# CVLAB-Unibo/Real-time-self-adaptive-deep-stereo

Hardware: AMD Instinct MI355X
Metric: adapted stereo pairs/sec (whole node), MADNet full-backprop online adaptation 1242x375 (higher is better)
Workload: dtype bf16 MFMA operands, f32 accumulate/storage (forward: split-bf16 = 3 MFMAs per product on the large 3x3 layers, exact f32 MFMA on the others, so the disparity stays within 1e-3 px; gradients: plain bf16); 1 GPU; MADNet FULL adaptation step (fwd+SSIM/L1 loss+EPE+bwd+momentum), 1242x375, 1 pair/GPU/step, private model per stream; precision=mixed, launch=hipGraph replay, step_sync=stream, concurrent_private_streams_per_gpu=1

## Files before the change

real-time-self-adaptive-deep-stereo_amd/csrc/conv_patch.hip:

```cpp
#include "conv_args.h"
#include <stdlib.h>
#include <algorithm>
#include <atomic>

namespace {

struct PatchGeo {
    int TH, tiles_y, tiles_x, ntiles_n, nwg;
    int KP, CPT, PS;
    int nchunk;
    int patch_halfs;
    float inv_kp4;
    unsigned mul_kp8;
    int dbg;
    mh_tile_decode dec;
    mh_fastdiv f_kp4, f_pc;
    int xuse, per, n_major;
    mh_fastdiv f_pt;
};

constexpr int LSB = 80;
constexpr int PW = 18;

template <int WM, int WN, int MT, int NT, bool DGRAD, int CPTC = 0, bool X3 = false>
__global__ __launch_bounds__(WM * WN * 64) __attribute__((amdgpu_waves_per_eu(1, 2))) void conv_patch_kernel(ConvArgs p, PatchGeo g) {
    static_assert(!X3 || !DGRAD, "the split-bf16 instances are forward only");
    constexpr int NTH = WM * WN * 64;
    constexpr int BM = WM * MT * 16, BN = WN * NT * 16;
    constexpr int TH = BM / 16;
    HIP_DYNAMIC_SHARED(float, smem_all)
    unsigned short* const Ph = reinterpret_cast<unsigned short*>(smem_all);
    unsigned short* const Bh = Ph + (X3 ? 2 : 1) * g.patch_halfs;
    constexpr int BLO = 2 * BN * LSB;
    const int tid = threadIdx.x, lane = tid & 63, wave = tid >> 6;
    const int wm = wave / WN, wn = wave % WN;
    const int li = lane & 15, lq = lane >> 4;
    const int d = p.dil;

    const int lin = mh_xcd_remap(blockIdx.x, g.nwg);
    int tile_n, ttx, tty, cx, cy, b;
    mh_decode_tile(lin, g.dec, tile_n, ttx, tty, cx, cy, b);
    const int n0 = tile_n * BN;
    const int y00 = cy + d * (tty * TH), x00 = cx + d * (ttx * 16);

    const __amdgpu_buffer_rsrc_t rs_in = mh_make_rsrc(p.in, p.in_bytes);
    const __amdgpu_buffer_rsrc_t rs_w = mh_make_rsrc(p.w, p.w_bytes);

    constexpr int FU = 512 / NTH;
    constexpr int DI = (16 * BN) / NTH;
    constexpr int NB = DGRAD ? DI : 4 * FU;
    constexpr int NV = DGRAD ? DI : FU;
    float4 rb0[NB], rb1[NB];
    int voff[NV], vk[NV], vch[NV];
#pragma unroll
    for (int jj = 0; jj < NV; ++jj) {
        const int q = tid + NTH * jj;
        if (!DGRAD) {
            const int wi = q & 255;
            const int n4 = wi % (BN / 4), kq = wi / (BN / 4);
            const int n = n0 + n4 * 4;
            vch[jj] = __builtin_amdgcn_readfirstlane(q >> 8);
            vk[jj] = kq * 4;
            voff[jj] = (kq < 8 && n < p.N) ? (kq * 4 * p.N + n) * 4 : MH_OOB;
        } else {
            const int ch = q / (8 * BN), rem = q - ch * (8 * BN);
            const int nn = rem >> 3, kg = rem & 7;
            vch[jj] = ch;
            vk[jj] = kg * 4;
            voff[jj] = (n0 + nn < p.N) ? ((n0 + nn) * p.K + kg * 4) * 4 : MH_OOB;
        }
    }
// ... 561 lines not shown
            __builtin_amdgcn_sched_barrier(0);
        }
    }
    __syncthreads();

    constexpr int CS = BN + 4;
    float* const Cs = smem_all;
#pragma unroll
    for (int i = 0; i < MT; ++i)
#pragma unroll
        for (int j = 0; j < NT; ++j)
#pragma unroll
            for (int r = 0; r < 4; ++r)
                Cs[((wm * MT + i) * 16 + lq * 4 + r) * CS + wn * NT * 16 + j * 16 + li] = acc[i][j][r];
    __syncthreads();
    constexpr int C4 = BN / 4;
    constexpr int RP = NTH / C4;
    constexpr int PASSES = (BM + RP - 1) / RP;
    const __amdgpu_buffer_rsrc_t rs_out = mh_make_rsrc(p.out, p.out_bytes);
    const __amdgpu_buffer_rsrc_t rs_mask = mh_make_rsrc(p.mask_ref ? p.mask_ref : p.out, p.mask_ref ? p.mask_bytes : 0u);
    const int c4 = tid % C4;
    const int n = n0 + c4 * 4;
    float4 bv = make_float4(0.f, 0.f, 0.f, 0.f);
    if (p.bias && n < p.N) bv = *reinterpret_cast<const float4*>(p.bias + n);
#pragma unroll 4
    for (int ps = 0; ps < PASSES; ++ps) {
        const int row = tid / C4 + ps * RP;
        const int rr = row < BM ? row : 0;
        const int y = y00 + (rr >> 4) * d, x = x00 + (rr & 15) * d;
        const bool ok = (tid < RP * C4) && (row < BM) && (y < p.Ho) && (x < p.Wo) && (n < p.N);
        const int m = (b * p.Ho + y) * p.Wo + x;
        float4 v = *reinterpret_cast<const float4*>(&Cs[rr * CS + c4 * 4]);
        const int ooff = ok ? (m * p.out_ld + n) * 4 : MH_OOB;
        float4 old = make_float4(0.f, 0.f, 0.f, 0.f), mk = make_float4(1.f, 1.f, 1.f, 1.f);
        if (p.accumulate) old = mh_buf_load4(rs_out, ooff);
        if (p.mask_ref) mk = mh_buf_load4(rs_mask, ok ? (m * p.mask_ld + n) * 4 : MH_OOB);
        v.x += bv.x; v.y += bv.y; v.z += bv.z; v.w += bv.w;
        if (p.alpha != 1.0f) {
            v.x = v.x > 0.f ? v.x : p.alpha * v.x; v.y = v.y > 0.f ? v.y : p.alpha * v.y;
            v.z = v.z > 0.f ? v.z : p.alpha * v.z; v.w = v.w > 0.f ? v.w : p.alpha * v.w;
        }
        v.x += old.x; v.y += old.y; v.z += old.z; v.w += old.w;
        if (p.mask_ref) {
            v.x *= (mk.x > 0.f || n + 0 < p.mask_c0 || n + 0 >= p.mask_c1) ? 1.0f : p.mask_alpha;
            v.y *= (mk.y > 0.f || n + 1 < p.mask_c0 || n + 1 >= p.mask_c1) ? 1.0f : p.mask_alpha;
            v.z *= (mk.z > 0.f || n + 2 < p.mask_c0 || n + 2 >= p.mask_c1) ? 1.0f : p.mask_alpha;
            v.w *= (mk.w > 0.f || n + 3 < p.mask_c0 || n + 3 >= p.mask_c1) ? 1.0f : p.mask_alpha;
        }
        if (ok) *reinterpret_cast<float4*>(p.out + (int64_t)m * p.out_ld + n) = v;
        if (ok && p.shadow) *reinterpret_cast<uint2*>(p.shadow + (int64_t)m * p.shadow_ld + n) = make_uint2(mh_pack_bf16(v.x, v.y), mh_pack_bf16(v.z, v.w));
    }
}

template <bool DGRAD, int PL>
__global__ __launch_bounds__(1024) void conv_bank_small_kernel(ConvArgs p, PatchGeo g) {
    constexpr int NTH = 1024, TH = 2, BM = 32, BN = 32, MT = 2, NT = 2, NCH = 4;
    HIP_DYNAMIC_SHARED(float, smem_all)
    unsigned short* const Ph = reinterpret_cast<unsigned short*>(smem_all);
    const int tid = threadIdx.x, lane = tid & 63, wave = tid >> 6;
    const int li = lane & 15, lq = lane >> 4;
    const int d = p.dil;
    const int st = DGRAD ? 1 : p.stride;
    const int PC = st * 16 + 3 - st;

    int lin;
    if (g.xuse < 8) {
        const int xcd = (int)blockIdx.x & 7, idx = (int)blockIdx.x >> 3;
        lin = xcd * g.per + idx;
        if (xcd >= g.xuse || lin >= g.nwg) return;
    } else lin = mh_xcd_remap(blockIdx.x, g.nwg);
    int tile_n, ttx, tty, cx, cy, b;
    if (g.n_major) {
        const int tn = mh_fdiv(lin, g.f_pt);
        mh_decode_tile(lin - tn * (int)g.f_pt.d, g.dec, tile_n, ttx, tty, cx, cy, b);
        tile_n = tn;
    } else mh_decode_tile(lin, g.dec, tile_n, ttx, tty, cx, cy, b);
    const int n0 = tile_n * BN;
    const int y00 = cy + d * (tty * TH), x00 = cx + d * (ttx * 16);

    const __amdgpu_buffer_rsrc_t rs_in = mh_make_rsrc(p.in, p.in_bytes);
    const __amdgpu_buffer_rsrc_t rs_b = mh_make_rsrc(p.wb, p.wb_bytes);

    const int my_n = n0 + (tid & 31);
    const int my_row = tid >> 5;
    const int my_y = y00 + (my_row >> 4) * d, my_x = x00 + (my_row & 15) * d;
    const bool my_ok = my_y < p.Ho && my_x < p.Wo && my_n < p.N;
    const int64_t my_m = ((int64_t)b * p.Ho + my_y) * p.Wo + my_x;
    const __amdgpu_buffer_rsrc_t rs_bias = mh_make_rsrc(p.bias ? (const void*)p.bias : (const void*)p.in, p.bias ? (unsigned)(p.N * 4) : 0u);
    const __amdgpu_buffer_rsrc_t rs_old = mh_make_rsrc(p.out, p.accumulate ? p.out_bytes : 0u);
    const __amdgpu_buffer_rsrc_t rs_mk = mh_make_rsrc(p.mask_ref ? (const void*)p.mask_ref : (const void*)p.in, p.mask_ref ? p.mask_bytes : 0u);
    float my_bias, my_old, my_mk;
    const int np16 = (p.N + 15) >> 4;
    const int stride_b = np16 * PL * 1024;
    u32x4 fb[NCH][NT][PL];
#pragma unroll
    for (int c = 0; c < NCH; ++c) {
        const int q = wave + 16 * c;
#pragma unroll
        for (int j = 0; j < NT; ++j) {
            const int nt = tile_n * (BN / 16) + j;
            const int off = (q < g.nchunk && nt < np16) ? q * stride_b + nt * PL * 1024 + lane * 16 : MH_OOB;
#pragma unroll
            for (int pl = 0; pl < PL; ++pl) fb[c][j][pl] = __builtin_amdgcn_raw_buffer_load_b128(rs_b, off == MH_OOB ? MH_OOB : off + pl * 1024, 0, 0);
        }
    }

    {
        constexpr int U = 4, ROUNDS = 2;
        const int kp4 = g.KP >> 2;
        const int items = (st * TH + 3 - st) * PC * kp4;
        auto fdiv = [](int n, const mh_fastdiv& f) { const int h = (int)__umulhi((unsigned)n, f.m); return f.d > 1 ? h : n; };
#pragma unroll
        for (int rd = 0; rd < ROUNDS; ++rd) {
            if (rd > 0 && items <= rd * U * NTH) break;
            float4 wv[U];
            int ldsv[U], c4v[U];
#pragma unroll
            for (int u = 0; u < U; ++u) {
                const int q = tid + (rd * U + u) * NTH;
                const int pp = fdiv(q, g.f_kp4), c4 = q - pp * kp4;
                const int pi = fdiv(pp, g.f_pc), pj = pp - pi * PC;
                const int iy = y00 * st - p.pad_t + pi * d, ix = x00 * st - p.pad_l + pj * d;
                const bool ok = q < items && (unsigned)iy < (unsigned)p.Hi && (unsigned)ix < (unsigned)p.Wi && (c4 < p.G);
                int off = (((b * p.Hi + iy) * p.Wi + ix) * p.in_ld + c4 * 4) * 4;
                MH_KEEP_VGPR(off);
                wv[u] = mh_buf_load4(rs_in, ok ? off : MH_OOB);
                ldsv[u] = q < items ? pp * g.PS + c4 * 4 : -1;
                c4v[u] = c4;
            }
            if (rd == 0) {
                my_bias = mh_buf_load1(rs_bias, my_n < p.N ? my_n * 4 : MH_OOB);
                my_old = mh_buf_load1(rs_old, my_ok ? (int)((my_m * p.out_ld + my_n) * 4) : MH_OOB);
                my_mk = mh_buf_load1(rs_mk, my_ok ? (int)((my_m * p.mask_ld + my_n) * 4) : MH_OOB);
            }
#pragma unroll
            for (int u = 0; u < U; ++u) {
                float4 w = wv[u];
                const int c4 = c4v[u];
                w.y = (c4 * 4 + 1 < p.K) ? w.y : 0.f;
                w.z = (c4 * 4 + 2 < p.K) ? w.z : 0.f;
                w.w = (c4 * 4 + 3 < p.K) ? w.w : 0.f;
                const int lds = ldsv[u];
                if (lds >= 0) {
                    if constexpr (PL == 2) {
                        uint2 hi, lo;
                        mh_split_bf16x2(w.x, w.y, hi.x, lo.x);
                        mh_split_bf16x2(w.z, w.w, hi.y, lo.y);
                        *reinterpret_cast<uint2*>(Ph + lds) = hi;
                        *reinterpret_cast<uint2*>(Ph + g.patch_halfs + lds) = lo;
                    } else
                    *reinterpret_cast<uint2*>(Ph + lds) = make_uint2(mh_pack_bf16(w.x, w.y), mh_pack_bf16(w.z, w.w));
                }
            }
        }
    }
    __syncthreads();

    f32x4 acc[MT][NT];
#pragma unroll
    for (int i = 0; i < MT; ++i)
#pragma unroll
        for (int j = 0; j < NT; ++j) acc[i][j] = (f32x4){0.f, 0.f, 0.f, 0.f};
    const unsigned short* const Pw = Ph + (li * st) * g.PS + lq * 8;
#pragma unroll
    for (int c = 0; c < NCH; ++c) {
        const int q = wave + 16 * c;
        if (q < g.nchunk) {
            const int tap = q / g.CPT, c32 = q - tap * g.CPT;
            const int ky = tap / 3, kx = tap - ky * 3;
            const int oy = DGRAD ? 2 - ky : ky, ox = DGRAD ? 2 - kx : kx;
            const unsigned short* Ab = Pw + (oy * PC + ox) * g.PS + c32 * 32;
            u32x4 fa[MT][PL];
#pragma unroll
            for (int i = 0; i < MT; ++i)
#pragma unroll
                for (int pl = 0; pl < PL; ++pl) fa[i][pl] = *reinterpret_cast<const u32x4*>(Ab + pl * g.patch_halfs + (i * st) * PC * g.PS);
#pragma unroll
            for (int t = (PL == 2 ? 0 : 2); t < 3; ++t)
#pragma unroll
                for (int i = 0; i < MT; ++i)
#pragma unroll
                    for (int j = 0; j < NT; ++j)
                        acc[i][j] = mh_mfma_bf16(fa[i][t == 0 ? PL - 1 : 0], fb[c][j][t == 1 ? PL - 1 : 0], acc[i][j]);
        }
    }
    __syncthreads();
    constexpr int CS = BN + 1;
    float* const Cs = smem_all;
#pragma unroll
    for (int i = 0; i < MT; ++i)
#pragma unroll
        for (int j = 0; j < NT; ++j)
#pragma unroll
            for (int r = 0; r < 4; ++r)
                Cs[(wave * BM + i * 16 + lq * 4 + r) * CS + j * 16 + li] = acc[i][j][r];
    __syncthreads();
    {
        const int row = tid >> 5, col = tid & 31;
        float v = 0.f;
#pragma unroll
        for (int w = 0; w < 16; ++w) v += Cs[(w * BM + row) * CS + col];
        const int n = n0 + col;
        if (my_ok) {
            const int64_t m = my_m;
            v += my_bias;
            if (p.alpha != 1.0f) v = v > 0.f ? v : p.alpha * v;
            float* dst = p.out + m * p.out_ld + n;
            v += my_old;
            if (p.mask_ref) v *= (my_mk > 0.f || n < p.mask_c0 || n >= p.mask_c1) ? 1.0f : p.mask_alpha;
            *dst = v;
            if (p.shadow) p.shadow[m * p.shadow_ld + n] = (unsigned short)mh_pack_bf16(v, 0.f);
        }
    }
}

__global__ __launch_bounds__(256) void pack_weights_kernel(const mh_pack_seg* __restrict__ segs, int nseg) {
    const int lo = mh_find_seg(segs, nseg, (int)blockIdx.x);
    const mh_pack_seg sg = segs[lo];
    const int e = ((int)blockIdx.x - sg.blk0) * 256 + (int)threadIdx.x;
    const int lane = e & 63, qt = e >> 6;
    if (sg.trans == 2 || sg.trans == 3) {
        const int k16 = (sg.K + 15) >> 4, nt32 = (sg.N + 31) >> 5;
        const int kc = sg.kc16 > 0 ? sg.kc16 : k16, nch = (k16 + kc - 1) / kc;
        if (qt >= nch * sg.taps * kc * nt32) return;
        const int nt = qt % nt32, q = qt / nt32;
        const int st = q % kc, q2 = q / kc;
        const int tap = q2 % sg.taps, ch = q2 / sg.taps;
        const int k0 = (ch * kc + st) * 16 + (lane >> 5) * 8, n = nt * 32 + (lane & 31);
        const int ts = sg.trans == 3 ? sg.taps - 1 - tap : tap;
        float v[8];
#pragma unroll
        for (int j = 0; j < 8; ++j)
            v[j] = (k0 + j < sg.K && n < sg.N) ? (sg.trans == 3 ? sg.src[((int64_t)ts * sg.N + n) * sg.K + k0 + j] : sg.src[((int64_t)ts * sg.K + k0 + j) * sg.N + n]) : 0.f;
        unsigned hh[4], ll[4];
#pragma unroll
        for (int j = 0; j < 4; ++j) mh_split_bf16x2(v[2 * j], v[2 * j + 1], hh[j], ll[j]);
        const int pln = (sg.trans == 3 || sg.planes < 2) ? 1 : 2;
        u32x4* dst = reinterpret_cast<u32x4*>(sg.dst) + (int64_t)qt * (64 * pln) + lane;
        dst[0] = (u32x4){hh[0], hh[1], hh[2], hh[3]};
        if (pln == 2) dst[64] = (u32x4){ll[0], ll[1], ll[2], ll[3]};
        return;
    }
    const int cpt = (sg.K + 31) >> 5, np16 = (sg.N + 15) >> 4;
    if (qt >= sg.taps * cpt * np16) return;
    const int nt = qt % np16, q = qt / np16;
    const int c = q % cpt, tap = q / cpt;
    const int k0 = c * 32 + (lane >> 4) * 8, n = nt * 16 + (lane & 15);
    float v[8];
#pragma unroll
    for (int j = 0; j < 8; ++j)
        v[j] = (k0 + j < sg.K && n < sg.N) ? (sg.trans ? sg.src[((int64_t)tap * sg.N + n) * sg.K + k0 + j] : sg.src[((int64_t)tap * sg.K + k0 + j) * sg.N + n]) : 0.f;
    unsigned hh[4], ll[4];
#pragma unroll
    for (int j = 0; j < 4; ++j) mh_split_bf16x2(v[2 * j], v[2 * j + 1], hh[j], ll[j]);
    const u32x4 h = {hh[0], hh[1], hh[2], hh[3]}, l = {ll[0], ll[1], ll[2], ll[3]};
    u32x4* dst = reinterpret_cast<u32x4*>(sg.dst) + ((int64_t)qt * sg.planes) * 64 + lane;
    dst[0] = h;
    if (sg.planes > 1) dst[64] = l;
}

constexpr size_t PATCH_LDS_MAX = 150 * 1024;

size_t patch_lds(int TH, int BM, int BN, int KP, bool x3 = false) {
    const size_t tiles = ((size_t)(TH + 2) * PW * (KP + 16) * 2 + (size_t)2 * BN * LSB * 2) * (x3 ? 2 : 1);
    const size_t cs = (size_t)BM * (BN + 4) * 4;
    return tiles > cs ? tiles : cs;
}

size_t bank_lds(int TH, int BM, int BN, int KP, bool x3) {
    const size_t patch = (size_t)(TH + 2) * PW * (KP + 16) * 2 * (x3 ? 2 : 1);
    const size_t cs = (size_t)BM * (BN + 4) * 4;
    return patch > cs ? patch : cs;
}

constexpr int PATCH_DEFAULT = 1;
std::atomic<int> g_patch_mode{-2};
int patch_mode() {
    int m = g_patch_mode.load(std::memory_order_relaxed);
    if (m == -2) { const char* e = getenv("MH_CONV_PATCH"); m = e ? atoi(e) : PATCH_DEFAULT; g_patch_mode.store(m, std::memory_order_relaxed); }
    return m;
}
std::atomic<int> g_patch_launches{0};

template <int WM, int WN, int MT, int NT, bool DGRAD, int CPTC = 0, bool X3 = false>
int launch_patch(ConvArgs& a, hipStream_t s) {
    constexpr int BM = WM * MT * 16, BN = WN * NT * 16, TH = BM / 16;
    static std::atomic<uint64_t> attr_done{0};
    if (int rc = mh_lds_optin(attr_done, reinterpret_cast<const void*>(&conv_patch_kernel<WM, WN, MT, NT, DGRAD, CPTC, X3>), (int)PATCH_LDS_MAX, "conv_patch")) return rc;
    if (a.M < 0) return 0;
    PatchGeo g;
    g.TH = TH;
    const int d = a.dil;
    g.tiles_y = mh_cdiv(mh_cdiv(a.Ho, d), TH);
    g.tiles_x = mh_cdiv(mh_cdiv(a.Wo, d), 16);
    g.ntiles_n = mh_cdiv(a.N, BN);
    g.nwg = a.B * d * d * g.tiles_y * g.tiles_x * g.ntiles_n;
    {
        const int64_t nwg64 = (int64_t)g.nwg;
        const int dmax = std::max(std::max(g.ntiles_n, g.tiles_x), std::max(g.tiles_y, (int)d));
        MH_REQUIRE(mh_fastdiv_ok(nwg64, dmax), MH_ERR_UNSUPPORTED, "tile decode: %lld workgroups x divisor %d exceeds the 2^32 range of the magic-multiplier division", (long long)nwg64, dmax);
    }
    g.dec = mh_make_tile_decode(g.ntiles_n, g.tiles_x, g.tiles_y, d);
    g.KP = (a.K + 31) & ~31;
    g.CPT = g.KP / 32;
    g.PS = g.KP + 16;
    g.nchunk = 9 * g.CPT;
    g.patch_halfs = (TH + 2) * PW * g.PS;
    g.inv_kp4 = 1.0f / (float)(g.KP / 4);
    g.mul_kp8 = (unsigned)(((1ull << 32) + (g.KP / 8) - 1) / (g.KP / 8));
    g.dbg = (patch_mode() >> 9) & 3;
    const size_t lds = patch_lds(TH, BM, BN, g.KP, X3);
    ++g_patch_launches;
    mh_note_kernel("conv_patch_kernel<%d,%d,%d,%d,%s,CPTC=%d,%s> tile %dx%d K=%d dil=%d grid %d lds %d", WM, WN, MT, NT, DGRAD ? "dgrad" : "fwd", CPTC,
                   X3 ? "bf16x3" : "bf16", BM, BN, a.K, a.dil, g.nwg, (int)lds);
    hipLaunchKernelGGL((conv_patch_kernel<WM, WN, MT, NT, DGRAD, CPTC, X3>), dim3(g.nwg), dim3(WM * WN * 64), lds, s, a, g);
    return mh_check_launch("conv_patch");
}

std::atomic<int> g_bank_launches{0};
template <int WM, int WN, int MT, int NT, bool X3>
int launch_bank(ConvArgs& a, hipStream_t s) {
    constexpr int BM = WM * MT * 16, BN = WN * NT * 16, TH = BM / 16;
    static std::atomic<uint64_t> attr_done{0};
    if (int rc = mh_lds_optin(attr_done, reinterpret_cast<const void*>(&conv_bank_kernel<WM, WN, MT, NT, X3>), (int)PATCH_LDS_MAX, "conv_bank")) return rc;
    if (a.M < 0) return 0;
    PatchGeo g;
    g.TH = TH;
    const int d = a.dil;
    g.tiles_y = mh_cdiv(mh_cdiv(a.Ho, d), TH);
    g.tiles_x = mh_cdiv(mh_cdiv(a.Wo, d), 16);
    g.ntiles_n = mh_cdiv(a.N, BN);
    g.nwg = a.B * d * d * g.tiles_y * g.tiles_x * g.ntiles_n;
    {
        const int64_t nwg64 = (int64_t)g.nwg;
        const int dmax = std::max(std::max(g.ntiles_n, g.tiles_x), std::max(g.tiles_y, (int)d));
        MH_REQUIRE(mh_fastdiv_ok(nwg64, dmax), MH_ERR_UNSUPPORTED, "tile decode: %lld workgroups x divisor %d exceeds the 2^32 range of the magic-multiplier division", (long long)nwg64, dmax);
    }
    g.dec = mh_make_tile_decode(g.ntiles_n, g.tiles_x, g.tiles_y, d);
    g.KP = (a.K + 31) & ~31;
    g.CPT = g.KP / 32;
    g.PS = g.KP + 16;
    g.nchunk = 9 * g.CPT;
    g.patch_halfs = (TH + 2) * PW * g.PS;
    g.inv_kp4 = 1.0f / (float)(g.KP / 4);
    g.mul_kp8 = (unsigned)(((1ull << 32) + (g.KP / 8) - 1) / (g.KP / 8));
    g.dbg = (patch_mode() >> 9) & 3;
    const size_t lds = bank_lds(TH, BM, BN, g.KP, X3);
    ++g_patch_launches;
    ++g_bank_launches;
    mh_note_kernel("conv_bank_kernel<%d,%d,%d,%d,%s> tile %dx%d K=%d dil=%d grid %d lds %d", WM, WN, MT, NT, X3 ? "bf16x3" : "bf16", BM, BN, a.K, a.dil,
                   g.nwg, (int)lds);
    hipLaunchKernelGGL((conv_bank_kernel<WM, WN, MT, NT, X3>), dim3(g.nwg), dim3(WM * WN * 64), lds, s, a, g);
    return mh_check_launch("conv_bank");
}

std::atomic<int> g_bank_small_place{-1};
template <bool DGRAD, int PL>
int launch_bank_small(ConvArgs& a, hipStream_t s) {
    static std::atomic<uint64_t> attr_done{0};
    if (int rc = mh_lds_optin(attr_done, reinterpret_cast<const void*>(&conv_bank_small_kernel<DGRAD, PL>), (int)PATCH_LDS_MAX, "conv_bank_small")) return rc;
    if (a.M < 0) return 0;
    PatchGeo g;
    g.TH = 2;
    const int d = a.dil;
    g.tiles_y = mh_cdiv(mh_cdiv(a.Ho, d), 2);
    g.tiles_x = mh_cdiv(mh_cdiv(a.Wo, d), 16);
    g.ntiles_n = mh_cdiv(a.N, 32);
    g.nwg = a.B * d * d * g.tiles_y * g.tiles_x * g.ntiles_n;
    {
        const int64_t nwg64 = (int64_t)g.nwg;
        const int dmax = std::max(std::max(g.ntiles_n, g.tiles_x), std::max(g.tiles_y, (int)d));
        MH_REQUIRE(mh_fastdiv_ok(nwg64, dmax), MH_ERR_UNSUPPORTED, "tile decode: %lld workgroups x divisor %d exceeds the 2^32 range of the magic-multiplier division", (long long)nwg64, dmax);
    }
    g.KP = (a.K + 31) & ~31;
    {
        const int mode_raw = g_bank_small_place.load(std::memory_order_relaxed);
        const int mode = mode_raw < 0 ? 1 : mode_raw;
        const int npt = g.nwg / g.ntiles_n;
        int X = 8;
        if (mode >= 2) { X = 1; while (X < 8 && mh_cdiv(g.nwg, X) > 32) X *= 2; }
        const double bank = 9.0 * g.KP * a.N * 2.0 * PL, in = (double)a.B * (DGRAD ? a.Ho : a.Hi) * (DGRAD ? a.Wo : a.Wi) * a.K * 4.0;
        const double pix_major = X * bank + in;
        const double col_major = (double)std::max(X, g.ntiles_n) / g.ntiles_n * bank + std::min(X, g.ntiles_n) * in;
        g.n_major = (mode != 0 && mode != 2 && col_major < pix_major) ? 1 : 0;
        g.xuse = X;
        g.per = mh_cdiv(g.nwg, X);
        g.f_pt = mh_make_fastdiv(npt);
        MH_REQUIRE(mh_fastdiv_ok((int64_t)g.nwg, npt), MH_ERR_UNSUPPORTED, "tile decode: %d workgroups x %d pixel tiles exceeds the magic-multiplier range", g.nwg, npt);
    }
    g.dec = mh_make_tile_decode(g.n_major ? 1 : g.ntiles_n, g.tiles_x, g.tiles_y, d);
    g.CPT = g.KP / 32;
    g.PS = g.KP + 16;
    g.nchunk = 9 * g.CPT;
    const int st = DGRAD ? 1 : a.stride;
    g.patch_halfs = (st * 2 + 3 - st) * (st * 16 + 3 - st) * g.PS;
    g.f_kp4 = mh_make_fastdiv(g.KP / 4); g.f_pc = mh_make_fastdiv(st * 16 + 3 - st);
    g.inv_kp4 = 1.0f / (float)(g.KP / 4);
    g.mul_kp8 = (unsigned)(((1ull << 32) + (g.KP / 8) - 1) / (g.KP / 8));
    g.dbg = 0;
    const size_t patch = (size_t)g.patch_halfs * 2 * PL, cs = (size_t)16 * 32 * 33 * 4;
    const size_t lds = patch > cs ? patch : cs;
    ++g_bank_launches;
    const int nblocks = g.xuse < 8 ? 8 * g.per : g.nwg;
    mh_note_kernel("conv_bank_small_kernel<%s,%s> tile 32x32 K=%d N=%d dil=%d grid %d lds %d", DGRAD ? "dgrad" : "fwd", PL == 2 ? "bf16x3" : "bf16", a.K, a.N, a.dil,
                   g.nwg, (int)lds);
    hipLaunchKernelGGL((conv_bank_small_kernel<DGRAD, PL>), dim3(nblocks), dim3(1024), lds, s, a, g);
    return mh_check_launch("conv_bank_small");
}

template <int WM, int WN, int MT, int NT, bool DGRAD>
int launch_patch_k(ConvArgs& a, hipStream_t s) {
    const bool all = a.M < 0;
    const bool generic = !all && ((patch_mode() >> 11) & 1) != 0;
    int rc = 0;
    if constexpr (WM == 4) {
        if (all || (a.K == 128 && !generic)) { rc = launch_patch<WM, WN, MT, NT, DGRAD, 4>(a, s); if (!all || rc) return rc; }
        if (all || (a.K == 64 && !generic)) { rc = launch_patch<WM, WN, MT, NT, DGRAD, 2>(a, s); if (!all || rc) return rc; }
    }
    return launch_patch<WM, WN, MT, NT, DGRAD>(a, s);
}

template <int WM, int WN, int MT, bool DGRAD>
int launch_patch_n(ConvArgs& a, hipStream_t s, int bn) {
    const bool all = a.M < 0;
    int rc = 0;
    if (all || bn == 128) { rc = launch_patch_k<WM, WN, MT, 4, DGRAD>(a, s); if (!all || rc) return rc; }
    if (all || bn == 96) { rc = launch_patch_k<WM, WN, MT, 3, DGRAD>(a, s); if (!all || rc) return rc; }
    if (all || bn == 64) { rc = launch_patch_k<WM, WN, MT, 2, DGRAD>(a, s); if (!all || rc) return rc; }
    return rc;
}

int patch_bn(const ConvArgs& a) {
    if (a.N <= 32) return 32;
    return a.x3 ? (a.N > 64 ? 128 : 64) : (a.N > 96 ? 128 : (a.N > 64 ? 96 : 64));
}

int patch_bm(const ConvArgs& a) {
    if (a.x3) return a.N > 64 ? 64 : 128;
    if ((patch_mode() & 0xff) == 64 || (patch_mode() & 0xff) == 128) return patch_mode() & 0xff;
    return 128;
}
bool patch_w8(const ConvArgs& a) { return (patch_mode() & 0xff) == 1 ? true : (patch_mode() & 0x100) != 0; }

}

extern "C" int mh_tune_conv_patch(int mode) {
    g_patch_mode = mode < 0 ? PATCH_DEFAULT : mode;
    return g_patch_launches.exchange(0);
}

extern "C" int64_t mh_pack_bytes(int32_t taps, int32_t K, int32_t N, int32_t planes) {
    return (int64_t)taps * ((K + 31) / 32) * ((N + 15) / 16) * planes * 1024;
}
extern "C" int mh_pack_weights(const mh_pack_seg* segs_device, int32_t nseg, int32_t nblocks, void* stream) {
    MH_REQUIRE(segs_device && nseg > 0 && nblocks > 0, MH_ERR_ARG, "mh_pack_weights: empty segment table");
    hipLaunchKernelGGL(pack_weights_kernel, dim3(nblocks), dim3(256), 0, (hipStream_t)stream, segs_device, nseg);
    return mh_check_launch("pack_weights");
}
std::atomic<int> g_bank_small_maxpix{-2};
// ... 113 lines not shown
```

real-time-self-adaptive-deep-stereo_amd/madnet_hip/ops.py:

```python
import ctypes as C
import torch
from . import _ffi


def same_pad(in_size, k, stride=1, dilation=1):
    keff = (k - 1) * dilation + 1
    out = -(-in_size // stride)
    total = max((out - 1) * stride + keff - in_size, 0)
    return out, total // 2, total - total // 2


class View(object):
    __slots__ = ("t", "ptr", "B", "H", "W", "C", "ld")

    def __init__(self, t, B, H, W, C_, ld, coff=0):
        self.t, self.B, self.H, self.W, self.C, self.ld = t, B, H, W, C_, ld
        self.ptr = t.data_ptr() + 4 * coff

    @property
    def npix(self):
        return self.B * self.H * self.W

    def slice(self, c0, c1):
        v = View(self.t, self.B, self.H, self.W, c1 - c0, self.ld)
# ... 75 lines not shown
    return conv_desc(dx.B, Ho, Wo, dx.H, dx.W, cout, cin, kh, kw_, stride, dil, pt, pl, 1, 1, dz.ld, dx.ld,
                     precision=(_bwd_precision() if precision is None else precision), **kw)


def conv2d_takes_bank(qlib, x, w, out, stride, dil, mode, precision, mask_ref=None):
    d = (_dgrad_desc if mode else _fwd_desc)(x, w, out, stride, dil, precision, mask_ld=(mask_ref.ld if mask_ref is not None else 0))
    return qlib.conv2d_takes_bank(C.byref(d), _p(x), _p(w), _p(out), _p(mask_ref)) == 1


def conv2d_fwd(lib, x, w, b, out, stride=1, dil=1, alpha=1.0, accumulate=False, mask_ref=None, mask_alpha=1.0,
               mask_range=(0, 0), stream=None, precision=None, wb=None, shadow=None, out_planes=None):
    d = _fwd_desc(x, w, out, stride, dil, precision, alpha=alpha, mask_ld=(mask_ref.ld if mask_ref is not None else 0), accumulate=int(accumulate),
                  mask_alpha=mask_alpha, mask_c0=mask_range[0], mask_c1=mask_range[1])
    if out_planes is not None:
        assert (out_planes.B, out_planes.H, out_planes.W, out_planes.C) == (out.B, out.H, out.W, out.C)
        lib.conv2d_sh4(C.byref(d), _p(x), _p(w), _p(wb), _p(b), _p(out), _p(mask_ref), C.c_void_p(out_planes.hi.ptr), C.c_void_p(out_planes.lo.ptr), _p(stream))
    elif shadow is not None:
        assert (shadow.B, shadow.H, shadow.W, shadow.C) == (out.B, out.H, out.W, out.C)
        lib.conv2d_sh(C.byref(d), _p(x), _p(w), _p(wb), _p(b), _p(out), _p(mask_ref), C.c_void_p(shadow.ptr), _p(stream))
    elif wb is not None:
        lib.conv2d_wb(C.byref(d), _p(x), _p(w), _p(wb), _p(b), _p(out), _p(mask_ref), _p(stream))
    else:
        lib.conv2d(C.byref(d), _p(x), _p(w), _p(b), _p(out), _p(mask_ref), _p(stream))


PLANES_WHOLE_MAX = int(__import__("os").environ.get("MH_PLANES_WHOLE_MAX", "8"))


def planes_kc16(K):
    k16 = (K + 15) // 16
    return 0 if (k16 <= PLANES_WHOLE_MAX or k16 == 13) else 4


def check_planes_rule(qlib):
    for K in (16, 97, 112, 128, 129, 193, 208, 256, 385, 1025):
        if int(qlib.planes_kc16(K)) != planes_kc16(K):
            raise RuntimeError("libmadnet_hip: mh_planes_kc16(%d) = %d, host rule %d (MH_PLANES_WHOLE_MAX mismatch)" % (K, qlib.planes_kc16(K), planes_kc16(K)))


def _k16_padded(K):
    k16, kc = (K + 15) // 16, planes_kc16(K)
    return (k16 + kc - 1) // kc * kc if kc else k16


def pack_bytes(w, planes=2, trans=0):
    kh, kw, K, N = w.shape
    if trans == 2:
        return kh * kw * _k16_padded(K) * ((N + 31) // 32) * 1024 * planes
    if trans == 3:
        return kh * kw * _k16_padded(N) * ((K + 31) // 32) * 1024
    if trans:
        K, N = N, K
    return kh * kw * ((K + 31) // 32) * ((N + 15) // 16) * planes * 1024


def pack_weights(lib, pairs, device, keep, stream=None):
    if not pairs:
        return
    arr = (_ffi.PackSeg * len(pairs))()
    blk = 0
    for i, pr in enumerate(pairs):
        src, dst = pr[0], pr[1]
        planes = pr[2] if len(pr) > 2 else 2
        trans = pr[3] if len(pr) > 3 else 0
        kh, kw, K, N = src.shape
        if trans in (1, 3):
            K, N = N, K
        assert dst.numel() * dst.element_size() >= pack_bytes(src, planes, trans) and dst.data_ptr() % 16 == 0
        assert (trans != 3 or planes == 1)
        arr[i].src, arr[i].dst, arr[i].taps, arr[i].K, arr[i].N = src.data_ptr(), dst.data_ptr(), kh * kw, K, N
        arr[i].planes, arr[i].blk0, arr[i].trans = planes, blk, trans
        arr[i].kc16 = planes_kc16(K) if trans in (2, 3) else 0
        if trans in (2, 3):
            blk += (kh * kw * _k16_padded(K) * ((N + 31) // 32) * 64 + 255) // 256
        else:
            blk += (kh * kw * ((K + 31) // 32) * ((N + 15) // 16) * 64 + 255) // 256
    table = torch.frombuffer(bytearray(bytes(arr)), dtype=torch.uint8).to(device)
    keep.append(table)
    lib.pack_weights(C.c_void_p(table.data_ptr()), len(pairs), blk, _p(stream))


def conv2d_dgrad(lib, dz, w, dx, stride=1, dil=1, accumulate=False, mask_ref=None, mask_alpha=1.0, mask_range=(0, 0),
                 stream=None, wb=None, shadow=None, dz_shadow=None, mask_shadow=None):
    d = _dgrad_desc(dz, w, dx, stride, dil, None, mask_ld=(mask_ref.ld if mask_ref is not None else 0), accumulate=int(accumulate),
                    mask_alpha=mask_alpha, mask_c0=mask_range[0], mask_c1=mask_range[1])
    if dz_shadow is not None or mask_shadow is not None:
        assert dz_shadow is None or (dz_shadow.B, dz_shadow.H, dz_shadow.W, dz_shadow.C) == (dz.B, dz.H, dz.W, dz.C)
        assert mask_shadow is None or (mask_ref is not None and (mask_shadow.B, mask_shadow.H, mask_shadow.W, mask_shadow.C) == (dx.B, dx.H, dx.W, dx.C))
        assert shadow is None or (shadow.B, shadow.H, shadow.W, shadow.C) == (dx.B, dx.H, dx.W, dx.C)
        sp = lambda sh: C.c_void_p(sh.ptr) if sh is not None else None
        lib.conv2d_sh3(C.byref(d), _p(dz), sp(dz_shadow), _p(w), _p(wb), None, _p(dx), _p(mask_ref), sp(mask_shadow), sp(shadow), 0, _p(stream))
    elif shadow is not None:
        assert (shadow.B, shadow.H, shadow.W, shadow.C) == (dx.B, dx.H, dx.W, dx.C)
        lib.conv2d_sh(C.byref(d), _p(dz), _p(w), _p(wb), None, _p(dx), _p(mask_ref), C.c_void_p(shadow.ptr), _p(stream))
    elif wb is not None:
        lib.conv2d_wb(C.byref(d), _p(dz), _p(w), _p(wb), None, _p(dx), _p(mask_ref), _p(stream))
    else:
        lib.conv2d(C.byref(d), _p(dz), _p(w), None, _p(dx), _p(mask_ref), _p(stream))


def conv2d_wgrad(lib, x, dz, dw, db, stride=1, dil=1, stream=None):
    kh, kw, cin, cout = dw.shape
    Ho, Wo, pt, pl = conv_geometry(x.H, x.W, kh, kw, stride, dil)
    assert (dz.H, dz.W, dz.C) == (Ho, Wo, cout) and x.C == cin
    d = conv_desc(x.B, x.H, x.W, Ho, Wo, cin, cout, kh, kw, stride, dil, pt, pl, 0, 0, x.ld, dz.ld, precision=_bwd_precision())
    lib.conv2d_wgrad(C.byref(d), _p(x), _p(dz), dz.ld, _p(dw), _p(db), _p(stream))


class WgradWorkspace(object):
    CHUNK = 64 << 20

    def __init__(self, device):
        self.device = device
        self.chunks = []
        self.reset()

    def reset(self):
        self.ci, self.off = 0, 0

    def alloc(self, nfloats):
        nfloats = (nfloats + 3) // 4 * 4
        while True:
            if self.ci == len(self.chunks):
                self.chunks.append(torch.empty(max(self.CHUNK, nfloats), dtype=torch.float32, device=self.device))
                self.off = 0
            c = self.chunks[self.ci]
            if self.off + nfloats <= c.numel():
                p = c.data_ptr() + 4 * self.off
                self.off += nfloats
# ... 610 lines not shown
```

Measured before the change: 769.5 pairs/s.

## Tile weight packing through LDS and add an optional multi-tile bank_small kernel

The weight-pack kernel now stages 32x128 tiles of the f32 weights in shared memory, reading them with coalesced float4 loads when alignment allows, before splitting into bf16 hi/lo planes. Previously each thread gathered eight strided scalars, and in the transposed layouts those reads were poorly coalesced. Separately, the small-bank conv kernel is refactored into a per-tile device function. A MULTI variant can then keep the B fragments in registers and loop over several spatial tiles, capping the grid at one residency round. That variant is enabled only when a placement flag bit is set. The host block-count formula changes to match the new pack grid, and the two sides must stay in sync.

```diff
diff --git a/real-time-self-adaptive-deep-stereo_amd/csrc/conv_patch.hip b/real-time-self-adaptive-deep-stereo_amd/csrc/conv_patch.hip
--- a/real-time-self-adaptive-deep-stereo_amd/csrc/conv_patch.hip
+++ b/real-time-self-adaptive-deep-stereo_amd/csrc/conv_patch.hip
@@ -17,6 +17,8 @@
     mh_fastdiv f_kp4, f_pc;
     int xuse, per, n_major;
     mh_fastdiv f_pt;
+    int tiles;
+    mh_fastdiv f_grp;
 };
 
 constexpr int LSB = 80;
@@ -684,37 +686,21 @@
     }
 }
 
-template <bool DGRAD, int PL>
-__global__ __launch_bounds__(1024) void conv_bank_small_kernel(ConvArgs p, PatchGeo g) {
+template <bool DGRAD, int PL, bool REMAT = false>
+__device__ __forceinline__ void bank_small_tile(const ConvArgs& p, const PatchGeo& g, float* const smem_all, const u32x4 (&fb)[4][2][PL], const int n0, const int y00,
+                                                const int x00, const int b, const __amdgpu_buffer_rsrc_t rs_in) {
     constexpr int NTH = 1024, TH = 2, BM = 32, BN = 32, MT = 2, NT = 2, NCH = 4;
-    HIP_DYNAMIC_SHARED(float, smem_all)
     unsigned short* const Ph = reinterpret_cast<unsigned short*>(smem_all);
-    const int tid = threadIdx.x, lane = tid & 63, wave = tid >> 6;
-    const int li = lane & 15, lq = lane >> 4;
+    const int tid = threadIdx.x, wave = tid >> 6;
+    int stid = tid;
+    if constexpr (REMAT) MH_KEEP_VGPR(stid);
+    const int li = stid & 15, lq = (stid & 63) >> 4;
     const int d = p.dil;
     const int st = DGRAD ? 1 : p.stride;
     const int PC = st * 16 + 3 - st;
 
-    int lin;
-    if (g.xuse < 8) {
-        const int xcd = (int)blockIdx.x & 7, idx = (int)blockIdx.x >> 3;
-        lin = xcd * g.per + idx;
-        if (xcd >= g.xuse || lin >= g.nwg) return;
-    } else lin = mh_xcd_remap(blockIdx.x, g.nwg);
-    int tile_n, ttx, tty, cx, cy, b;
-    if (g.n_major) {
-        const int tn = mh_fdiv(lin, g.f_pt);
-        mh_decode_tile(lin - tn * (int)g.f_pt.d, g.dec, tile_n, ttx, tty, cx, cy, b);
-        tile_n = tn;
-    } else mh_decode_tile(lin, g.dec, tile_n, ttx, tty, cx, cy, b);
-    const int n0 = tile_n * BN;
-    const int y00 = cy + d * (tty * TH), x00 = cx + d * (ttx * 16);
-
-    const __amdgpu_buffer_rsrc_t rs_in = mh_make_rsrc(p.in, p.in_bytes);
-    const __amdgpu_buffer_rsrc_t rs_b = mh_make_rsrc(p.wb, p.wb_bytes);
-
-    const int my_n = n0 + (tid & 31);
-    const int my_row = tid >> 5;
+    const int my_n = n0 + (stid & 31);
+    const int my_row = stid >> 5;
     const int my_y = y00 + (my_row >> 4) * d, my_x = x00 + (my_row & 15) * d;
     const bool my_ok = my_y < p.Ho && my_x < p.Wo && my_n < p.N;
     const int64_t my_m = ((int64_t)b * p.Ho + my_y) * p.Wo + my_x;
@@ -722,20 +708,6 @@
     const __amdgpu_buffer_rsrc_t rs_old = mh_make_rsrc(p.out, p.accumulate ? p.out_bytes : 0u);
     const __amdgpu_buffer_rsrc_t rs_mk = mh_make_rsrc(p.mask_ref ? (const void*)p.mask_ref : (const void*)p.in, p.mask_ref ? p.mask_bytes : 0u);
     float my_bias, my_old, my_mk;
-    const int np16 = (p.N + 15) >> 4;
-    const int stride_b = np16 * PL * 1024;
-    u32x4 fb[NCH][NT][PL];
-#pragma unroll
-    for (int c = 0; c < NCH; ++c) {
-        const int q = wave + 16 * c;
-#pragma unroll
-        for (int j = 0; j < NT; ++j) {
-            const int nt = tile_n * (BN / 16) + j;
-            const int off = (q < g.nchunk && nt < np16) ? q * stride_b + nt * PL * 1024 + lane * 16 : MH_OOB;
-#pragma unroll
-            for (int pl = 0; pl < PL; ++pl) fb[c][j][pl] = __builtin_amdgcn_raw_buffer_load_b128(rs_b, off == MH_OOB ? MH_OOB : off + pl * 1024, 0, 0);
-        }
-    }
 
     {
         constexpr int U = 4, ROUNDS = 2;
@@ -749,7 +721,7 @@
             int ldsv[U], c4v[U];
 #pragma unroll
             for (int u = 0; u < U; ++u) {
-                const int q = tid + (rd * U + u) * NTH;
+                const int q = stid + (rd * U + u) * NTH;
                 const int pp = fdiv(q, g.f_kp4), c4 = q - pp * kp4;
                 const int pi = fdiv(pp, g.f_pc), pj = pp - pi * PC;
                 const int iy = y00 * st - p.pad_t + pi * d, ix = x00 * st - p.pad_l + pj * d;
@@ -828,7 +800,7 @@
                 Cs[(wave * BM + i * 16 + lq * 4 + r) * CS + j * 16 + li] = acc[i][j][r];
     __syncthreads();
     {
-        const int row = tid >> 5, col = tid & 31;
+        const int row = stid >> 5, col = stid & 31;
         float v = 0.f;
 #pragma unroll
         for (int w = 0; w < 16; ++w) v += Cs[(w * BM + row) * CS + col];
@@ -846,49 +818,161 @@
     }
 }
 
+template <bool DGRAD, int PL, bool MULTI>
+__global__ __launch_bounds__(1024) void conv_bank_small_kernel(ConvArgs p, PatchGeo g) {
+    constexpr int TH = 2, BN = 32, NT = 2, NCH = 4;
+    HIP_DYNAMIC_SHARED(float, smem_all)
+    const int tid = threadIdx.x, lane = tid & 63, wave = tid >> 6;
+    const int d = p.dil;
+
+    int lin;
+    if (!MULTI && g.xuse < 8) {
+        const int xcd = (int)blockIdx.x & 7, idx = (int)blockIdx.x >> 3;
+        lin = xcd * g.per + idx;
+        if (xcd >= g.xuse || lin >= g.nwg) return;
+    } else lin = mh_xcd_remap(blockIdx.x, g.nwg);
+    int tile_n, ttx, tty, cx, cy, b;
+    int px = 0, cnt = 1;
+    if (MULTI) {
+        tile_n = mh_fdiv(lin, g.f_grp);
+        px = (lin - tile_n * (int)g.f_grp.d) * g.tiles;
+        cnt = min(g.tiles, (int)g.f_pt.d - px);
+        int tn0;
+        mh_decode_tile(px, g.dec, tn0, ttx, tty, cx, cy, b);
+    } else if (g.n_major) {
+        const int tn = mh_fdiv(lin, g.f_pt);
+        mh_decode_tile(lin - tn * (int)g.f_pt.d, g.dec, tile_n, ttx, tty, cx, cy, b);
+        tile_n = tn;
+    } else mh_decode_tile(lin, g.dec, tile_n, ttx, tty, cx, cy, b);
+    const int n0 = tile_n * BN;
+
+    const __amdgpu_buffer_rsrc_t rs_in = mh_make_rsrc(p.in, p.in_bytes);
+    const __amdgpu_buffer_rsrc_t rs_b = mh_make_rsrc(p.wb, p.wb_bytes);
+    const int np16 = (p.N + 15) >> 4;
+    const int stride_b = np16 * PL * 1024;
+    u32x4 fb[NCH][NT][PL];
+#pragma unroll
+    for (int c = 0; c < NCH; ++c) {
+        const int q = wave + 16 * c;
+#pragma unroll
+        for (int j = 0; j < NT; ++j) {
+            const int nt = tile_n * (BN / 16) + j;
+            const int off = (q < g.nchunk && nt < np16) ? q * stride_b + nt * PL * 1024 + lane * 16 : MH_OOB;
+#pragma unroll
+            for (int pl = 0; pl < PL; ++pl) fb[c][j][pl] = __builtin_amdgcn_raw_buffer_load_b128(rs_b, off == MH_OOB ? MH_OOB : off + pl * 1024, 0, 0);
+        }
+    }
+    constexpr bool PEEL = !(MULTI && PL == 2);
+    if constexpr (PEEL) bank_small_tile<DGRAD, PL>(p, g, smem_all, fb, n0, cy + d * (tty * TH), cx + d * (ttx * 16), b, rs_in);
+    if constexpr (MULTI) {
+#pragma nounroll
+        for (int t = PEEL ? 1 : 0; t < cnt; ++t) {
+            __syncthreads();
+            int tn0;
+            mh_decode_tile(px + t, g.dec, tn0, ttx, tty, cx, cy, b);
+            bank_small_tile<DGRAD, PL, !PEEL>(p, g, smem_all, fb, n0, cy + d * (tty * TH), cx + d * (ttx * 16), b, rs_in);
+        }
+    }
+}
+
+constexpr int PACK_ROWS = 32, PACK_RUN = 128;
 __global__ __launch_bounds__(256) void pack_weights_kernel(const mh_pack_seg* __restrict__ segs, int nseg) {
+    constexpr int P0 = PACK_RUN + 2, P1 = PACK_RUN + 4;
+    __shared__ __attribute__((aligned(16))) float T[PACK_ROWS * P1];
     const int lo = mh_find_seg(segs, nseg, (int)blockIdx.x);
     const mh_pack_seg sg = segs[lo];
-    const int e = ((int)blockIdx.x - sg.blk0) * 256 + (int)threadIdx.x;
-    const int lane = e & 63, qt = e >> 6;
-    if (sg.trans == 2 || sg.trans == 3) {
-        const int k16 = (sg.K + 15) >> 4, nt32 = (sg.N + 31) >> 5;
-        const int kc = sg.kc16 > 0 ? sg.kc16 : k16, nch = (k16 + kc - 1) / kc;
-        if (qt >= nch * sg.taps * kc * nt32) return;
-        const int nt = qt % nt32, q = qt / nt32;
-        const int st = q % kc, q2 = q / kc;
-        const int tap = q2 % sg.taps, ch = q2 / sg.taps;
-        const int k0 = (ch * kc + st) * 16 + (lane >> 5) * 8, n = nt * 32 + (lane & 31);
-        const int ts = sg.trans == 3 ? sg.taps - 1 - tap : tap;
+    const int tid = (int)threadIdx.x;
+    const bool img32 = sg.trans >= 2, ctg = (sg.trans & 1) != 0;
+    int kc = 0, k16p = 0, kp;
+    if (img32) {
+        const int k16 = (sg.K + 15) >> 4;
+        kc = sg.kc16 > 0 ? sg.kc16 : k16;
+        k16p = (k16 + kc - 1) / kc * kc;
+        kp = k16p * 16;
+    } else kp = ((sg.K + 31) >> 5) * 32;
+    const int nkb = ctg ? (kp + PACK_RUN - 1) / PACK_RUN : (kp + PACK_ROWS - 1) / PACK_ROWS;
+    const int nnb = ctg ? (sg.N + PACK_ROWS - 1) / PACK_ROWS : (sg.N + PACK_RUN - 1) / PACK_RUN;
+    const int sb = (int)blockIdx.x - sg.blk0;
+    const int nb = sb % nnb, kb = (sb / nnb) % nkb, tap = sb / (nnb * nkb);
+    if (tap >= sg.taps) return;
+    const int ts = sg.trans == 3 ? sg.taps - 1 - tap : tap;
+    const int R = ctg ? sg.N : sg.K, C = ctg ? sg.K : sg.N;
+    const int r0 = (ctg ? nb : kb) * PACK_ROWS, c0 = (ctg ? kb : nb) * PACK_RUN;
+    const float* const tsrc = sg.src + (int64_t)ts * R * C;
+    const int pitch = ctg ? P1 : P0;
+    if ((C & 3) == 0 && (reinterpret_cast<uintptr_t>(sg.src) & 15u) == 0) {
+        float4 v[4];
+#pragma unroll
+        for (int i = 0; i < 4; ++i) {
+            const int slot = tid + 256 * i, r = r0 + (slot >> 5), c = c0 + (slot & 31) * 4;
+            const bool ok = r < R && c < C;
+            v[i] = *reinterpret_cast<const float4*>(ok ? tsrc + (int64_t)r * C + c : sg.src);
+            if (!ok) v[i] = make_float4(0.f, 0.f, 0.f, 0.f);
+        }
+#pragma unroll
+        for (int i = 0; i < 4; ++i) {
+            const int slot = tid + 256 * i;
+            float* const d = T + (slot >> 5) * pitch + (slot & 31) * 4;
+            float2 a, b;
+            a.x = v[i].x; a.y = v[i].y; b.x = v[i].z; b.y = v[i].w;
+            *reinterpret_cast<float2*>(d) = a;
+            *reinterpret_cast<float2*>(d + 2) = b;
+        }
+    } else {
+        float v[16];
+#pragma unroll
+        for (int i = 0; i < 16; ++i) {
+            const int flat = tid + 256 * i, r = r0 + (flat >> 7), c = c0 + (flat & 127);
+            const bool ok = r < R && c < C;
+            v[i] = *(ok ? tsrc + (int64_t)r * C + c : sg.src);
+            if (!ok) v[i] = 0.f;
+        }
+#pragma unroll
+        for (int i = 0; i < 16; ++i) {
+            const int flat = tid + 256 * i;
+            T[(flat >> 7) * pitch + (flat & 127)] = v[i];
+        }
+    }
+    __syncthreads();
+    const int pln = (sg.trans == 3 || sg.planes < 2) ? 1 : 2;
+#pragma unroll
+    for (int i = 0; i < 2; ++i) {
+        const int o = tid + 256 * i, lane = o & 63, f = o >> 6;
+        int kl, nl, qt;
+        bool ok;
+        if (!img32) {
+            const int cpt = kp >> 5, np16 = (sg.N + 15) >> 4;
+            const int cl = ctg ? f >> 1 : 0, ntl = ctg ? f & 1 : f;
+            const int c = (ctg ? kb * 4 : kb) + cl, nt = (ctg ? nb * 2 : nb * 8) + ntl;
+            ok = c < cpt && nt < np16;
+            qt = (tap * cpt + c) * np16 + nt;
+            kl = cl * 32 + (lane >> 4) * 8; nl = ntl * 16 + (lane & 15);
+        } else {
+            const int nt32 = (sg.N + 31) >> 5;
+            const int sl = ctg ? f : f >> 2, ntl = ctg ? 0 : f & 3;
+            const int ks = (ctg ? kb * 8 : kb * 2) + sl, nt = (ctg ? nb : nb * 4) + ntl;
+            ok = ks < k16p && nt < nt32;
+            const int ch = ks / kc, st = ks - ch * kc;
+            qt = ((ch * sg.taps + tap) * kc + st) * nt32 + nt;
+            kl = sl * 16 + (lane >> 5) * 8; nl = ntl * 32 + (lane & 31);
+        }
         float v[8];
-#pragma unroll
-        for (int j = 0; j < 8; ++j)
-            v[j] = (k0 + j < sg.K && n < sg.N) ? (sg.trans == 3 ? sg.src[((int64_t)ts * sg.N + n) * sg.K + k0 + j] : sg.src[((int64_t)ts * sg.K + k0 + j) * sg.N + n]) : 0.f;
+        if (ctg) {
+            const float4 a = *reinterpret_cast<const float4*>(T + nl * P1 + kl), b = *reinterpret_cast<const float4*>(T + nl * P1 + kl + 4);
+            v[0] = a.x; v[1] = a.y; v[2] = a.z; v[3] = a.w; v[4] = b.x; v[5] = b.y; v[6] = b.z; v[7] = b.w;
+        } else {
+#pragma unroll
+            for (int j = 0; j < 8; ++j) v[j] = T[(kl + j) * P0 + nl];
+        }
         unsigned hh[4], ll[4];
 #pragma unroll
         for (int j = 0; j < 4; ++j) mh_split_bf16x2(v[2 * j], v[2 * j + 1], hh[j], ll[j]);
-        const int pln = (sg.trans == 3 || sg.planes < 2) ? 1 : 2;
-        u32x4* dst = reinterpret_cast<u32x4*>(sg.dst) + (int64_t)qt * (64 * pln) + lane;
-        dst[0] = (u32x4){hh[0], hh[1], hh[2], hh[3]};
-        if (pln == 2) dst[64] = (u32x4){ll[0], ll[1], ll[2], ll[3]};
-        return;
-    }
-    const int cpt = (sg.K + 31) >> 5, np16 = (sg.N + 15) >> 4;
-    if (qt >= sg.taps * cpt * np16) return;
-    const int nt = qt % np16, q = qt / np16;
-    const int c = q % cpt, tap = q / cpt;
-    const int k0 = c * 32 + (lane >> 4) * 8, n = nt * 16 + (lane & 15);
-    float v[8];
-#pragma unroll
-    for (int j = 0; j < 8; ++j)
-        v[j] = (k0 + j < sg.K && n < sg.N) ? (sg.trans ? sg.src[((int64_t)tap * sg.N + n) * sg.K + k0 + j] : sg.src[((int64_t)tap * sg.K + k0 + j) * sg.N + n]) : 0.f;
-    unsigned hh[4], ll[4];
-#pragma unroll
-    for (int j = 0; j < 4; ++j) mh_split_bf16x2(v[2 * j], v[2 * j + 1], hh[j], ll[j]);
-    const u32x4 h = {hh[0], hh[1], hh[2], hh[3]}, l = {ll[0], ll[1], ll[2], ll[3]};
-    u32x4* dst = reinterpret_cast<u32x4*>(sg.dst) + ((int64_t)qt * sg.planes) * 64 + lane;
-    dst[0] = h;
-    if (sg.planes > 1) dst[64] = l;
+        if (ok) {
+            u32x4* dst = reinterpret_cast<u32x4*>(sg.dst) + (int64_t)qt * (64 * pln) + lane;
+            dst[0] = (u32x4){hh[0], hh[1], hh[2], hh[3]};
+            if (pln == 2) dst[64] = (u32x4){ll[0], ll[1], ll[2], ll[3]};
+        }
+    }
 }
 
 constexpr size_t PATCH_LDS_MAX = 150 * 1024;
@@ -987,11 +1071,32 @@
 }
 
 std::atomic<int> g_bank_small_place{-1};
+int bank_small_round(const void* kernel, size_t lds, int nwg) {
+#ifdef __HIPCC__
+    static std::atomic<int> cus[64];
+    int dev = 0;
+    if (hipGetDevice(&dev) != hipSuccess) dev = 0;
+    int n = cus[dev & 63].load(std::memory_order_relaxed);
+    if (n == 0) {
+        if (hipDeviceGetAttribute(&n, hipDeviceAttributeMultiprocessorCount, dev) != hipSuccess || n <= 0) { (void)hipGetLastError(); return nwg; }
+        cus[dev & 63].store(n, std::memory_order_relaxed);
+    }
+    if (nwg <= n) return n;
+    int per = 0;
+    if (hipOccupancyMaxActiveBlocksPerMultiprocessor(&per, kernel, 1024, lds) != hipSuccess || per < 1) { (void)hipGetLastError(); per = 1; }
+    return n * per;
+#else
+    (void)kernel; (void)lds; (void)nwg;
+    return 256;
+#endif
+}
 template <bool DGRAD, int PL>
 int launch_bank_small(ConvArgs& a, hipStream_t s) {
-    static std::atomic<uint64_t> attr_done{0};
-    if (int rc = mh_lds_optin(attr_done, reinterpret_cast<const void*>(&conv_bank_small_kernel<DGRAD, PL>), (int)PATCH_LDS_MAX, "conv_bank_small")) return rc;
+    static std::atomic<uint64_t> attr_done{0}, attr_done_multi{0};
+    if (int rc = mh_lds_optin(attr_done, reinterpret_cast<const void*>(&conv_bank_small_kernel<DGRAD, PL, false>), (int)PATCH_LDS_MAX, "conv_bank_small")) return rc;
+    if (int rc = mh_lds_optin(attr_done_multi, reinterpret_cast<const void*>(&conv_bank_small_kernel<DGRAD, PL, true>), (int)PATCH_LDS_MAX, "conv_bank_small")) return rc;
     if (a.M < 0) return 0;
+    const int place_raw = g_bank_small_place.load(std::memory_order_relaxed);
     PatchGeo g;
     g.TH = 2;
     const int d = a.dil;
@@ -1006,8 +1111,7 @@
     }
     g.KP = (a.K + 31) & ~31;
     {
-        const int mode_raw = g_bank_small_place.load(std::memory_order_relaxed);
-        const int mode = mode_raw < 0 ? 1 : mode_raw;
+        const int mode = place_raw < 0 ? 1 : (place_raw & 3);
         const int npt = g.nwg / g.ntiles_n;
         int X = 8;
         if (mode >= 2) { X = 1; while (X < 8 && mh_cdiv(g.nwg, X) > 32) X *= 2; }
@@ -1033,10 +1137,26 @@
     const size_t patch = (size_t)g.patch_halfs * 2 * PL, cs = (size_t)16 * 32 * 33 * 4;
     const size_t lds = patch > cs ? patch : cs;
     ++g_bank_launches;
+    const int npt = g.nwg / g.ntiles_n, ntiles = g.nwg;
+    g.tiles = 1;
+    g.f_grp = mh_make_fastdiv(npt);
+    if (place_raw >= 0 && (place_raw & 4)) {
+        const int round = bank_small_round(reinterpret_cast<const void*>(&conv_bank_small_kernel<DGRAD, PL, true>), lds, g.nwg);
+        if (g.nwg > round) {
+            int T = 2;
+            while (T < npt && (int64_t)g.ntiles_n * mh_cdiv(npt, T) > round) ++T;
+            g.tiles = T;
+            g.f_grp = mh_make_fastdiv(mh_cdiv(npt, T));
+            g.nwg = g.ntiles_n * mh_cdiv(npt, T);
+            g.n_major = 1; g.xuse = 8; g.per = mh_cdiv(g.nwg, 8);
+            g.dec = mh_make_tile_decode(1, g.tiles_x, g.tiles_y, d);
+        }
+    }
     const int nblocks = g.xuse < 8 ? 8 * g.per : g.nwg;
-    mh_note_kernel("conv_bank_small_kernel<%s,%s> tile 32x32 K=%d N=%d dil=%d grid %d lds %d", DGRAD ? "dgrad" : "fwd", PL == 2 ? "bf16x3" : "bf16", a.K, a.N, a.dil,
-                   g.nwg, (int)lds);
-    hipLaunchKernelGGL((conv_bank_small_kernel<DGRAD, PL>), dim3(nblocks), dim3(1024), lds, s, a, g);
+    mh_note_kernel("conv_bank_small_kernel<%s,%s> tile 32x32 K=%d N=%d dil=%d grid %d lds %d tiles %d", DGRAD ? "dgrad" : "fwd", PL == 2 ? "bf16x3" : "bf16", a.K, a.N,
+                   a.dil, ntiles, (int)lds, g.tiles);
+    if (g.tiles > 1) hipLaunchKernelGGL((conv_bank_small_kernel<DGRAD, PL, true>), dim3(nblocks), dim3(1024), lds, s, a, g);
+    else hipLaunchKernelGGL((conv_bank_small_kernel<DGRAD, PL, false>), dim3(nblocks), dim3(1024), lds, s, a, g);
     return mh_check_launch("conv_bank_small");
 }
 
diff --git a/real-time-self-adaptive-deep-stereo_amd/madnet_hip/ops.py b/real-time-self-adaptive-deep-stereo_amd/madnet_hip/ops.py
--- a/real-time-self-adaptive-deep-stereo_amd/madnet_hip/ops.py
+++ b/real-time-self-adaptive-deep-stereo_amd/madnet_hip/ops.py
@@ -151,6 +151,17 @@
     if trans:
         K, N = N, K
     return kh * kw * ((K + 31) // 32) * ((N + 15) // 16) * planes * 1024
+
+
+def pack_blocks(taps, K, N, trans, kc16=None):
+    if trans in (2, 3) and kc16 is not None:
+        k16 = (K + 15) // 16
+        kpad = ((k16 + kc16 - 1) // kc16 * kc16 if kc16 else k16) * 16
+    else:
+        kpad = _k16_padded(K) * 16 if trans in (2, 3) else (K + 31) // 32 * 32
+    if trans in (1, 3):
+        return taps * ((kpad + 127) // 128) * ((N + 31) // 32)
+    return taps * ((kpad + 31) // 32) * ((N + 127) // 128)
 
 
 def pack_weights(lib, pairs, device, keep, stream=None):
@@ -170,10 +181,7 @@
         arr[i].src, arr[i].dst, arr[i].taps, arr[i].K, arr[i].N = src.data_ptr(), dst.data_ptr(), kh * kw, K, N
         arr[i].planes, arr[i].blk0, arr[i].trans = planes, blk, trans
         arr[i].kc16 = planes_kc16(K) if trans in (2, 3) else 0
-        if trans in (2, 3):
-            blk += (kh * kw * _k16_padded(K) * ((N + 31) // 32) * 64 + 255) // 256
-        else:
-            blk += (kh * kw * ((K + 31) // 32) * ((N + 15) // 16) * 64 + 255) // 256
+        blk += pack_blocks(kh * kw, K, N, trans)
     table = torch.frombuffer(bytearray(bytes(arr)), dtype=torch.uint8).to(device)
     keep.append(table)
     lib.pack_weights(C.c_void_p(table.data_ptr()), len(pairs), blk, _p(stream))
```

New measurement: 774.1 pairs/s, median of 6. Within noise of the previous version (+0.6%).
